# kiranchhatre/amuse

Measured on AMD Instinct MI355X. Metric: SMPL-X frames/sec (10 s clip, 1000-step DDPM), higher is better.
Workload: dtype bf16; 1 GPU; 256 x 10 s clips in total (256 on rank 0), DDPM-1000 sampling loop + VAE decode (300 frames) + 6D->axis-angle; random-init weights of the diff_latent_v2 / prior_emotional_fing architecture; clips_total=256, clips_rank0=256, clips_per_tile=2, sampler=ddpm-1000, mfma_operands=bf16, state_and_accumulate=fp32

## Files before the change

### amuse_amd/csrc/k_vae_fusedx.hip

```cpp
#define AMUSE_OP_F16
#include "amuse_fused.hpp"

namespace amuse {
namespace {

constexpr int kXKvBytes = 4 * kKeyRows * 64;
constexpr int kXOffKv = 0;
constexpr int kXOffW = kXOffKv + kXKvBytes;
constexpr int kXOffPv = kXOffW + kWBufs * kStageBytes;
constexpr int kXOffCa = kXOffPv + 2 * kPvSlot;
constexpr int kXLdsBytes = kXOffCa + kCaBytes;
static_assert(kXLdsBytes <= 160 * 1024, "LDS");
constexpr int kParkTile = 8192;

__device__ __forceinline__ f32x4 mfma3(f16x8 wh, f16x8 wl, const F16Pair& x, f32x4 acc) {
    acc = mfma_f16(wl, x.hi, acc);
    acc = mfma_f16(wh, x.lo, acc);
    return mfma_f16(wh, x.hi, acc);
}
__device__ __forceinline__ f32x4 mfma3t(f16x8 wh, f16x8 wl, const F16Pair& x, f32x4 acc) {
    acc = mfma_f16(x.hi, wl, acc);
    acc = mfma_f16(x.lo, wh, acc);
    return mfma_f16(x.hi, wh, acc);
}
constexpr int kP = 2;
template <int NT>
__device__ __forceinline__ void stage_fetch_x(Stager& s) {
    const unsigned d = __builtin_amdgcn_readfirstlane(s.dst0 + s.widx * kStageBytes);
#pragma unroll
    for (int i = 0; i < kP; ++i) glds16(s.src + i * 64, d + i * 1024);
    s.src += kStage * 64;
    s.widx = s.widx == kWBufs - 1 ? 0 : s.widx + 1;
}
template <int NT>
__device__ __forceinline__ void stage_end_x(Stager& s) {
    asm volatile("s_waitcnt vmcnt(%0) lgkmcnt(0)\n\ts_barrier" ::"n"(kP) : "memory");
    s.ridx = s.ridx == kWBufs - 1 ? 0 : s.ridx + 1;
}
template <int NT, bool FETCH = true, class F>
__device__ __forceinline__ void for_pairs(Stager& s, F&& f) {
    if constexpr (FETCH) stage_fetch_x<NT>(s);
    f16x8 h = wfrag(s, 0), l = wfrag(s, 1);
#pragma unroll
    for (int i = 0; i < 8; ++i) {
        const f16x8 ch = h, cl = l;
        if (i + 1 < 8) { h = wfrag(s, 2 * i + 2); l = wfrag(s, 2 * i + 3); }
        f(i, ch, cl);
    }
}

template <int NT>
struct Images {
    static constexpr int PARK = NT == 3 ? 2 : 0;
    F16Pair reg[NT - PARK][4];
    char* lds;
    __device__ __forceinline__ void build(const f32x4 (&x)[NT][kTiles]) {
#pragma unroll
        for (int j = 0; j < NT; ++j)
#pragma unroll
            for (int c = 0; c < 4; ++c) {
                const F16Pair p = split_f16(x[j][2 * c], x[j][2 * c + 1]);
                if (j < PARK) {
                    *reinterpret_cast<uint4*>(lds + j * kParkTile + (2 * c) * 1024) = __builtin_bit_cast(uint4, p.hi);
                    *reinterpret_cast<uint4*>(lds + j * kParkTile + (2 * c + 1) * 1024) = __builtin_bit_cast(uint4, p.lo);
                } else {
                    reg[j - PARK][c] = p;
                }
            }
    }
    __device__ __forceinline__ F16Pair get(int j, int c) const {
        if (j < PARK) {
            F16Pair p;
            p.hi = __builtin_bit_cast(f16x8, *reinterpret_cast<const uint4*>(lds + j * kParkTile + (2 * c) * 1024));
            p.lo = __builtin_bit_cast(f16x8, *reinterpret_cast<const uint4*>(lds + j * kParkTile + (2 * c + 1) * 1024));
            return p;
        }
        return reg[j - PARK][c];
    }
};

__device__ __forceinline__ void attend_x(const uint4* Kh, const uint4* Kl, const uint4* Vh, const uint4* Vl, const F16Pair& qs, f32x4 (&o)[2], int len, int g, int r) {
    const int fs = frag_slot(g, r);
    o[0] = o[1] = splat4(0.f);
    float m_run = 0.f;
    f32x4 os = splat4(0.f);
    const f16x8 ones = __builtin_bit_cast(f16x8, r == 0 ? uint4{OP_ONE2, OP_ONE2, OP_ONE2, OP_ONE2} : uint4{0u, 0u, 0u, 0u});
    auto pair = [&](int jp, auto first, auto masked) {
        constexpr bool FIRST = decltype(first)::value, MASKED = decltype(masked)::value;
        f16x8 kh[2], kl[2], vh[2], vl[2];
#pragma unroll
        for (int u = 0; u < 2; ++u) {
            kh[u] = __builtin_bit_cast(f16x8, Kh[(2 * jp + u) * 64 + fs]);
            kl[u] = __builtin_bit_cast(f16x8, Kl[(2 * jp + u) * 64 + fs]);
        }
#pragma unroll
        for (int u = 0; u < 2; ++u) {
            vh[u] = __builtin_bit_cast(f16x8, Vh[(2 * jp + u) * 64 + fs]);
            vl[u] = __builtin_bit_cast(f16x8, Vl[(2 * jp + u) * 64 + fs]);
        }
        f32x4 st[2];
        const f32x4 c0 = splat4(-m_run);
#pragma unroll
        for (int u = 0; u < 2; ++u) {
            st[u] = mfma_f16(kl[u], qs.hi, c0);
            st[u] = mfma_f16(kh[u], qs.lo, st[u]);
            st[u] = mfma_f16(kh[u], qs.hi, st[u]);
        }
        if constexpr (MASKED) {
            int lim = len - 32 * jp - 4 * g;
#pragma unroll
            for (int u = 0; u < 2; ++u)
#pragma unroll
                for (int m = 0; m < 4; ++m) st[u][m] = (16 * u + m < lim) ? st[u][m] : -INFINITY;
        }
        float mx = max3(max3(st[0][0], st[0][1], st[0][2]), max3(st[0][3], st[1][0], st[1][1]), fmaxf(st[1][2], st[1][3]));
        if (FIRST || __builtin_amdgcn_ballot_w64(mx > kAttnTau) != 0) {
            mx = allreduce_g_max(mx);
            const float d = FIRST ? mx : fmaxf(mx, 0.f);
            st[0] -= splat4(d);
            st[1] -= splat4(d);
            if constexpr (!FIRST) {
                const float alpha = __builtin_amdgcn_exp2f(-d);
                os *= alpha;
                o[0] *= alpha;
                o[1] *= alpha;
            }
            m_run += d;
        }
        f32x4 p[2];
#pragma unroll
        for (int u = 0; u < 2; ++u)
#pragma unroll
            for (int m = 0; m < 4; ++m) p[u][m] = __builtin_amdgcn_exp2f(st[u][m]);
        const F16Pair pp = split_f16(p[0], p[1]);
#pragma unroll
        for (int td = 0; td < 2; ++td) {
            o[td] = mfma_f16(vl[td], pp.hi, o[td]);
            o[td] = mfma_f16(vh[td], pp.lo, o[td]);
            o[td] = mfma_f16(vh[td], pp.hi, o[td]);
        }
        os = mfma_f16(ones, pp.lo, os);
        os = mfma_f16(ones, pp.hi, os);
    };
    const int full = min(len / 32, kPairs);
    if (full > 0) pair(0, std::true_type{}, std::false_type{});
    else pair(0, std::true_type{}, std::true_type{});
#pragma unroll 1
    for (int jp = 1; jp < full; ++jp) pair(jp, std::false_type{}, std::false_type{});
#pragma unroll 1
    for (int jp = max(full, 1); jp < kPairs; ++jp) pair(jp, std::false_type{}, std::true_type{});
    const float l = allreduce_g_sum(os[0]);
    o[0] = o[0] / l;
    o[1] = o[1] / l;
}

template <class A> struct Geo;
template <> struct Geo<VaeFusedXArgs> {
    static __device__ __forceinline__ int S(const VaeFusedXArgs&) { return kFrames; }
    static __device__ __forceinline__ float* tap(const VaeFusedXArgs& a) { return a.tap_out; }
    static __device__ __forceinline__ const float* c1(const VaeFusedXArgs& a) { return a.c1; }
    static __device__ __forceinline__ float* c1_out(const VaeFusedXArgs& a) { return a.c1_out; }
};
template <> struct Geo<DenFusedXArgs> {
    static __device__ __forceinline__ int S(const DenFusedXArgs& a) { return a.S; }
    static __device__ __forceinline__ float* tap(const DenFusedXArgs&) { return nullptr; }
    static __device__ __forceinline__ const float* c1(const DenFusedXArgs&) { return nullptr; }
    static __device__ __forceinline__ float* c1_out(const DenFusedXArgs&) { return nullptr; }
};

template <int NT, int MODE, class A>
__device__ __forceinline__ void attn_half_x(f32x4 (&x)[NT][kTiles], Stager& sg, const A& a, int b, int blk, int tile0, const float* pv, const float* pv_next_src, unsigned pv_next_dst,
                                            char* smem, int len, int wave, int lane) {
    const int g = lane >> 4, r = lane & 15;
    const int S = Geo<A>::S(a);
    const size_t nrows = (size_t)a.B * S, row0 = (size_t)b * S;
    [[maybe_unused]] const bool prof_on = blockIdx.x == 0 && threadIdx.x == 0 && (blk == 1 || blk == 6);
    FSTAMP(1);
    char* kv = smem + kXOffKv;
    Images<NT> im;
    im.lds = kv + (wave & 3) * (2 * kParkTile) + lane * 16;
    if constexpr (MODE == 2) {
        im.build(x);
        asm volatile("s_waitcnt lgkmcnt(0)" ::: "memory");
        const float* bias = a.pvec + PV_SKIP_B + (blk - 5) * kD;
#pragma unroll
        for (int j = 0; j < NT; ++j)
#pragma unroll
            for (int t = 0; t < kTiles; ++t) x[j][t] = ld4(bias + 16 * t + 4 * g);
#pragma unroll
        for (int c = 0; c < 4; ++c) {
            F16Pair xc[NT];
#pragma unroll
            for (int j = 0; j < NT; ++j) xc[j] = im.get(j, c);
            for_pairs<NT>(sg, [&](int o, f16x8 wh, f16x8 wl) {
#pragma unroll
                for (int j = 0; j < NT; ++j) x[j][o] = mfma3(wh, wl, xc[j], x[j][o]);
            });
            stage_end_x<NT>(sg);
        }
        const float* sk = a.skip + (size_t)(8 - blk) * nrows * kD;
#pragma unroll 1
        for (int c = 0; c < 4; ++c) {
            F16Pair xc[NT];
#pragma unroll
            for (int j = 0; j < NT; ++j) {
                const int frame = 16 * (tile0 + 4 * j) + r;
                const float* src = sk + (row0 + min(frame, S - 1)) * kD + 32 * c + 4 * g;
                const bool ok = frame < S;
                xc[j] = split_f16(ok ? ld4(src) : splat4(0.f), ok ? ld4(src + 16) : splat4(0.f));
            }
            for_pairs<NT>(sg, [&](int o, f16x8 wh, f16x8 wl) {
#pragma unroll
                for (int j = 0; j < NT; ++j) x[j][o] = mfma3(wh, wl, xc[j], x[j][o]);
            });
            stage_end_x<NT>(sg);
        }
    }
    FSTAMP(2);
    {
        uint4* Kh = reinterpret_cast<uint4*>(kv);
        uint4* Kl = Kh + kKeyRows * 4;
        uint4* Vh = Kl + kKeyRows * 4;
        uint4* Vl = Vh + kPairs * 2 * 16 * 4;
        float* obuf = (a.obuf + row0 * kD);
        constexpr float kScaling = 0.17677669529663687f, kLog2e = 1.44269504088896340736f;
#pragma unroll 1
        for (int h = 0; h < kHeads; ++h) {
            {
                f32x4 kk[NT][2], vv[NT][2];
                const f32x4 bk0 = ld4(pv + PV_IN_B + kD + 32 * h + 4 * g), bk1 = ld4(pv + PV_IN_B + kD + 32 * h + 16 + 4 * g);
                const float bv0 = pv[PV_IN_B + 2 * kD + 32 * h + r], bv1 = pv[PV_IN_B + 2 * kD + 32 * h + 16 + r];
#pragma unroll
                for (int j = 0; j < NT; ++j) {
                    kk[j][0] = bk0; kk[j][1] = bk1;
                    vv[j][0] = splat4(bv0); vv[j][1] = splat4(bv1);
                }
#pragma unroll
                for (int s2 = 0; s2 < 2; ++s2) {
                    F16Pair xc[NT];
                    for_pairs<NT>(sg, [&](int i, f16x8 wh, f16x8 wl) {
                        const int c = 2 * s2 + (i >> 2), t = i & 3;
                        if (t == 0) {
#pragma unroll
                            for (int j = 0; j < NT; ++j) xc[j] = split_f16(x[j][2 * c], x[j][2 * c + 1]);
                        }
#pragma unroll
                        for (int j = 0; j < NT; ++j) {
                            if (t < 2) kk[j][t] = mfma3(wh, wl, xc[j], kk[j][t]);
                            else vv[j][t - 2] = mfma3t(wh, wl, xc[j], vv[j][t - 2]);
                        }
                    });
                    if (s2 == 0) stage_end_x<NT>(sg);
                }
                FSTAMP(3);
#pragma unroll
                for (int j = 0; j < NT; ++j) {
                    const int tile = tile0 + 4 * j;
                    const bool ok = 16 * tile + r < S;
                    const F16Pair ks = split_f16(ok ? kk[j][0] : splat4(0.f), ok ? kk[j][1] : splat4(0.f));
                    Kh[tile * 64 + frag_slot(g, r)] = __builtin_bit_cast(uint4, ks.hi);
                    Kl[tile * 64 + frag_slot(g, r)] = __builtin_bit_cast(uint4, ks.lo);
#pragma unroll
                    for (int td = 0; td < 2; ++td) {
                        f32x4 v = vv[j][td];
#pragma unroll
                        for (int m = 0; m < 4; ++m) v[m] = (16 * tile + 4 * g + m < S) ? v[m] : 0.f;
                        const F16Pair vs = split_f16(v, v);
                        const int slot = ((tile >> 1) * 2 + td) * 64 + frag_slot(g, r);
                        const uint4 hi4 = __builtin_bit_cast(uint4, vs.hi), lo4 = __builtin_bit_cast(uint4, vs.lo);
                        *reinterpret_cast<uint2*>(reinterpret_cast<char*>(Vh + slot) + (tile & 1) * 8) = uint2{hi4.x, hi4.y};
                        *reinterpret_cast<uint2*>(reinterpret_cast<char*>(Vl + slot) + (tile & 1) * 8) = uint2{lo4.x, lo4.y};
                    }
                }
                FSTAMP(4);
                stage_end_x<NT>(sg);
                FSTAMP(5);
            }
            if (h == 0 && pv_next_src) {
                const unsigned d = __builtin_amdgcn_readfirstlane(pv_next_dst + wave * 1024);
                glds16(reinterpret_cast<const uint4*>(pv_next_src) + wave * 64 + lane, d);
            }
            F16Pair qs[NT];
            {
                f32x4 q[NT][2];
                const f32x4 bq0 = ld4(pv + PV_IN_B + 32 * h + 4 * g), bq1 = ld4(pv + PV_IN_B + 32 * h + 16 + 4 * g);
#pragma unroll
                for (int j = 0; j < NT; ++j) { q[j][0] = bq0; q[j][1] = bq1; }
                F16Pair xc[NT];
                for_pairs<NT>(sg, [&](int i, f16x8 wh, f16x8 wl) {
                    const int c = i >> 1, o = i & 1;
                    if (o == 0) {
#pragma unroll
                        for (int j = 0; j < NT; ++j) xc[j] = split_f16(x[j][2 * c], x[j][2 * c + 1]);
                    }
#pragma unroll
                    for (int j = 0; j < NT; ++j) q[j][o] = mfma3(wh, wl, xc[j], q[j][o]);
                });
#pragma unroll
                for (int j = 0; j < NT; ++j) qs[j] = split_f16((q[j][0] * kScaling) * kLog2e, (q[j][1] * kScaling) * kLog2e);
            }
            FSTAMP(6);
#pragma unroll 1
            for (int j = 0; j < NT; ++j) {
                f32x4 o[2];
                attend_x(Kh, Kl, Vh, Vl, qs[0], o, len, g, r);
                const int frame = 16 * (tile0 + 4 * j) + r;
                if (frame < S) {
                    float* dst = obuf + (size_t)frame * kD + 32 * h + 4 * g;
                    st4(dst, o[0]);
                    st4(dst + 16, o[1]);
                }
                const F16Pair first = qs[0];
#pragma unroll
                for (int jj = 0; jj + 1 < NT; ++jj) qs[jj] = qs[jj + 1];
                qs[NT - 1] = first;
            }
            FSTAMP(7);
            stage_end_x<NT>(sg);
            FSTAMP(8);
        }
    }
}

template <int NT, int MODE, bool ENCL, class A>
__device__ __forceinline__ void row_half_x(f32x4 (&x)[NT][kTiles], Stager& sg, const A& a, int blk, int tile0, int b, const float* pv, const float* cal, char* smem, int wave,
                                           int lane, const bool hoist = false) {
    const int g = lane >> 4, r = lane & 15;
    const int S = Geo<A>::S(a);
    const size_t nrows = (size_t)a.B * S, row0 = (size_t)b * S;
    [[maybe_unused]] const bool prof_on = blockIdx.x == 0 && threadIdx.x == 0 && (blk == 1 || blk == 6);
    char* kv = smem + kXOffKv;
    Images<NT> im;
    im.lds = kv + (wave & 3) * (2 * kParkTile) + lane * 16;
    if (hoist) {
#pragma unroll
        for (int j = 0; j < NT; ++j) {
            const int frame = 16 * (tile0 + 4 * j) + r;
#pragma unroll
            for (int t = 0; t < kTiles; ++t) x[j][t] = frame < S ? ld4(Geo<A>::c1(a) + (size_t)frame * kD + 16 * t + 4 * g) : splat4(0.f);
        }
    } else {
        float* obuf = (a.obuf + row0 * kD);
#pragma unroll
        for (int j = 0; j < NT; ++j)
#pragma unroll
            for (int t = 0; t < kTiles; ++t) x[j][t] += ld4(pv + PV_OUT_B + 16 * t + 4 * g);
        const unsigned obase = lds_addr(smem) + kXOffKv + (wave < 4 ? wave * 12288 : 49152 + (wave - 4) * 8192);
        const char* obuf_l = smem + kXOffKv + (wave < 4 ? wave * 12288 : 49152 + (wave - 4) * 8192) + lane * 16;
        const float* osrc[NT];
#pragma unroll
        for (int j = 0; j < NT; ++j) osrc[j] = obuf + (size_t)min(16 * (tile0 + 4 * j) + r, S - 1) * kD + 4 * g;
        auto fetch_o = [&](int c) {
            const unsigned d = __builtin_amdgcn_readfirstlane(obase + (c & 1) * (NT * 2048));
#pragma unroll
            for (int j = 0; j < NT; ++j) {
                glds16(reinterpret_cast<const uint4*>(osrc[j] + 32 * c), d + (2 * j) * 1024);
                glds16(reinterpret_cast<const uint4*>(osrc[j] + 32 * c + 16), d + (2 * j + 1) * 1024);
            }
        };
        fetch_o(0);
#pragma unroll 1
        for (int c = 0; c < 4; ++c) {
            stage_fetch_x<NT>(sg);
            if (c + 1 < 4) {
                fetch_o(c + 1);
                asm volatile("s_waitcnt vmcnt(%0)" ::"n"(kP + 2 * NT) : "memory");
            } else {
                asm volatile("s_waitcnt vmcnt(%0)" ::"n"(kP) : "memory");
            }
            F16Pair xc[NT];
#pragma unroll
            for (int j = 0; j < NT; ++j) {
                const char* src = obuf_l + (c & 1) * (NT * 2048) + (2 * j) * 1024;
                xc[j] = split_f16(*reinterpret_cast<const f32x4*>(src), *reinterpret_cast<const f32x4*>(src + 1024));
            }
            for_pairs<NT, false>(sg, [&](int o, f16x8 wh, f16x8 wl) {
#pragma unroll
                for (int j = 0; j < NT; ++j) x[j][o] = mfma3(wh, wl, xc[j], x[j][o]);
            });
            if (c + 1 < 4) {
                asm volatile("s_waitcnt vmcnt(%0) lgkmcnt(0)\n\ts_barrier" ::"n"(kP + 2 * NT) : "memory");
                sg.ridx = sg.ridx == kWBufs - 1 ? 0 : sg.ridx + 1;
            } else {
                stage_end_x<NT>(sg);
            }
            FSTAMP(9);
        }
    }
    {
        const float* ca = cal + blk * kD;
#pragma unroll 1
        for (int j = 0; j < NT; ++j) {
            if (!hoist) layer_norm_rows<false>(x[0], pv + PV_LN1_W, pv + PV_LN1_B, g);
            if (Geo<A>::c1_out(a) && blk == 0 && b == 0) {
                const int frame = 16 * (tile0 + 4 * j) + r;
                if (frame < S) {
#pragma unroll
                    for (int t = 0; t < kTiles; ++t) st4(Geo<A>::c1_out(a) + (size_t)frame * kD + 16 * t + 4 * g, x[0][t]);
                }
            }
            if constexpr (!ENCL) {
#pragma unroll
                for (int t = 0; t < kTiles; ++t) x[0][t] += ld4(ca + 16 * t + 4 * g);
                layer_norm_rows<false>(x[0], pv + PV_LN2_W, pv + PV_LN2_B, g);
            }
            rotate_tiles<NT>(x);
        }
    }
    FSTAMP(10);
    im.build(x);
    asm volatile("s_waitcnt lgkmcnt(0)" ::: "memory");
#pragma unroll
    for (int j = 0; j < NT; ++j)
#pragma unroll
        for (int t = 0; t < kTiles; ++t) x[j][t] += ld4(pv + PV_L2_B + 16 * t + 4 * g);
    f32x4 hid[NT][2];
    auto lin1 = [&](f32x4 (&acc)[NT][2], int ch) {
        const f32x4 b0 = ld4(pv + PV_L1_B + 32 * ch + 4 * g), b1 = ld4(pv + PV_L1_B + 32 * ch + 16 + 4 * g);
#pragma unroll
        for (int j = 0; j < NT; ++j) { acc[j][0] = b0; acc[j][1] = b1; }
        F16Pair xc[NT];
        for_pairs<NT>(sg, [&](int i, f16x8 wh, f16x8 wl) {
            const int c = i >> 1, o = i & 1;
            if (o == 0) {
#pragma unroll
                for (int j = 0; j < NT; ++j) xc[j] = im.get(j, c);
            }
#pragma unroll
            for (int j = 0; j < NT; ++j) {
                acc[j][o] = mfma3(wh, wl, xc[j], acc[j][o]);
            }
        });
    };
    auto gelu_split = [&](F16Pair (&hs)[NT]) {
#pragma unroll
        for (int j = 0; j < NT; ++j) {
#pragma unroll
            for (int i = 0; i < 2; ++i)
#pragma unroll
                for (int m = 0; m < 4; ++m) hid[j][i][m] = gelu_erf_bf(hid[j][i][m]);
            hs[j] = split_f16(hid[j][0], hid[j][1]);
        }
    };
    lin1(hid, 0);
    stage_end_x<NT>(sg);
#pragma unroll 1
    for (int ch = 0; ch < 16; ++ch) {
        F16Pair hs[NT];
        if (ch < 15) {
            f32x4 nxt[NT][2];
            FSTAMP(11);
            if constexpr (NT == 3) {
                lin1(nxt, ch + 1);
                __builtin_amdgcn_sched_barrier(0);
                gelu_split(hs);
            } else {
                gelu_split(hs);
                __builtin_amdgcn_sched_barrier(0);
                lin1(nxt, ch + 1);
            }
            FSTAMP(12);
            stage_end_x<NT>(sg);
            FSTAMP(13);
#pragma unroll
            for (int j = 0; j < NT; ++j) { hid[j][0] = nxt[j][0]; hid[j][1] = nxt[j][1]; }
        } else {
            gelu_split(hs);
        }
        for_pairs<NT>(sg, [&](int o, f16x8 wh, f16x8 wl) {
#pragma unroll
            for (int j = 0; j < NT; ++j) {
                x[j][o] = mfma3(wh, wl, hs[j], x[j][o]);
            }
        });
        FSTAMP(14);
        stage_end_x<NT>(sg);
        FSTAMP(15);
    }
#pragma unroll 1
    for (int j = 0; j < NT; ++j) {
        layer_norm_rows<false>(x[0], pv + (ENCL ? PV_LN2_W : PV_LN3_W), pv + (ENCL ? PV_LN2_B : PV_LN3_B), g);
        rotate_tiles<NT>(x);
    }
    FSTAMP(16);
    if constexpr (MODE == 0) {
        float* sk = a.skip + (size_t)blk * nrows * kD;
#pragma unroll
        for (int j = 0; j < NT; ++j) {
            const int frame = 16 * (tile0 + 4 * j) + r;
            if (frame < S) {
#pragma unroll
                for (int t = 0; t < kTiles; ++t) st4(sk + (row0 + frame) * kD + 16 * t + 4 * g, x[j][t]);
            }
        }
    }
    if (Geo<A>::tap(a) && b == 0) store_tap<NT>(Geo<A>::tap(a), blk, x, tile0, g, r);
}

template <int NT>
__device__ __forceinline__ void decode_tiles_x(const VaeFusedXArgs& a, char* smem, Stager& sg, int tile0, int b, int len, int wave, int lane) {
    const int g = lane >> 4, r = lane & 15;
    const float* pvl = reinterpret_cast<const float*>(smem + kXOffPv);
    const float* cal = reinterpret_cast<const float*>(smem + kXOffCa);
    const unsigned lds0 = lds_addr(smem);
    f32x4 x[NT][kTiles];
#pragma unroll
    for (int j = 0; j < NT; ++j) {
        const int frame = 16 * (tile0 + 4 * j) + r;
#pragma unroll
        for (int t = 0; t < kTiles; ++t) x[j][t] = frame < kFrames ? ld4(a.pe + (size_t)frame * kD + 16 * t + 4 * g) : splat4(0.f);
    }
    asm volatile("s_waitcnt vmcnt(2) lgkmcnt(0)\n\ts_barrier" ::: "memory");
    const bool hoist = a.c1 != nullptr && len == kFrames;
#pragma unroll 1
    for (int blk = 0; blk < 4; ++blk) {
        const float* pv = pvl + (blk & 1) * (kPvSlot / 4);
        const bool h0 = blk == 0 && hoist;
        if (h0) {
            const unsigned d = __builtin_amdgcn_readfirstlane(lds0 + kXOffPv + kPvSlot + wave * 1024);
            glds16(reinterpret_cast<const uint4*>(a.pvec + PV_BLOCK) + wave * 64 + lane, d);
        } else {
            attn_half_x<NT, 0>(x, sg, a, b, blk, tile0, pv, a.pvec + (blk + 1) * PV_BLOCK, lds0 + kXOffPv + ((blk + 1) & 1) * kPvSlot, smem, len, wave, lane);
        }
        row_half_x<NT, 0, false>(x, sg, a, blk, tile0, b, pv, cal, smem, wave, lane, h0);
    }
    attn_half_x<NT, 1>(x, sg, a, b, 4, tile0, pvl, a.pvec + 5 * PV_BLOCK, lds0 + kXOffPv + kPvSlot, smem, len, wave, lane);
    row_half_x<NT, 1, false>(x, sg, a, 4, tile0, b, pvl, cal, smem, wave, lane);
#pragma unroll 1
    for (int blk = 5; blk < kLayers; ++blk) {
        const float* pv = pvl + (blk & 1) * (kPvSlot / 4);
        attn_half_x<NT, 2>(x, sg, a, b, blk, tile0, pv, blk + 1 < kLayers ? a.pvec + (blk + 1) * PV_BLOCK : nullptr, lds0 + kXOffPv + ((blk + 1) & 1) * kPvSlot, smem, len, wave, lane);
        row_half_x<NT, 2, false>(x, sg, a, blk, tile0, b, pv, cal, smem, wave, lane);
    }
#pragma unroll 1
    for (int j = 0; j < NT; ++j) {
        layer_norm_rows<false>(x[0], a.pvec + PV_FINAL_W, a.pvec + PV_FINAL_B, g);
        rotate_tiles<NT>(x);
    }
    if (a.tap_out && b == 0) store_tap<NT>(a.tap_out, 9, x, tile0, g, r);
    F16Pair xs[NT][4];
#pragma unroll
    for (int j = 0; j < NT; ++j)
#pragma unroll
        for (int c = 0; c < 4; ++c) xs[j][c] = split_f16(x[j][2 * c], x[j][2 * c + 1]);
    float* fst = reinterpret_cast<float*>(smem + kXOffKv) + wave * 16 * kQStride;
#pragma unroll 1
    for (int quarter = 0; quarter < 4; ++quarter) {
        f32x4 f[NT][6];
#pragma unroll
        for (int o = 0; o < 6; ++o) {
            const f32x4 bi = ld4(a.final_bias + 16 * (6 * quarter + o) + 4 * g);
#pragma unroll
            for (int j = 0; j < NT; ++j) f[j][o] = bi;
        }
#pragma unroll
        for (int s3 = 0; s3 < 3; ++s3) {
            for_pairs<NT>(sg, [&](int i, f16x8 wh, f16x8 wl) {
                const int lin = 8 * s3 + i, c = lin / 6, o = lin - 6 * c;
#pragma unroll
                for (int j = 0; j < NT; ++j) f[j][o] = mfma3(wh, wl, xs[j][c], f[j][o]);
            });
            stage_end_x<NT>(sg);
        }
        const int f0 = 96 * quarter, nfe = quarter == 3 ? kFeats - 288 : 96, njo = quarter == 3 ? kJoints - 48 : 16;
#pragma unroll 1
        for (int j = 0; j < NT; ++j) {
            const int tile = tile0 + 4 * j;
            const int frame = 16 * tile + r;
            const bool keep = frame < kFrames && frame < len;
            const int rows_here = min(16, kFrames - 16 * tile);
            const size_t row0 = (size_t)b * kFrames + 16 * tile;
#pragma unroll
            for (int o = 0; o < 6; ++o) st4(fst + r * kQStride + 16 * o + 4 * g, keep ? f[0][o] : splat4(0.f));
            asm volatile("s_waitcnt lgkmcnt(0)" ::: "memory");
            if (a.feats_out) {
                for (int i = lane; i < rows_here * nfe; i += 64) {
                    const int rr = i / nfe, c = i - rr * nfe;
                    a.feats_out[(row0 + rr) * kFeats + f0 + c] = fst[rr * kQStride + c];
                }
            }
            if (a.poses_out) {
                for (int i = lane; i < rows_here * njo; i += 64) {
                    const int rr = i / njo, jn = i - rr * njo;
                    float aa[3];
                    rot6d_to_axis_angle(fst + rr * kQStride + 6 * jn, a.quat_mode, aa);
                    float* dst = a.poses_out + ((row0 + rr) * kJoints + 16 * quarter + jn) * 3;
                    dst[0] = aa[0]; dst[1] = aa[1]; dst[2] = aa[2];
                }
            }
            if (a.trans_out && quarter == 3) {
                for (int i = lane; i < rows_here * 3; i += 64) {
                    const int rr = i / 3, c = i - rr * 3;
                    a.trans_out[(row0 + rr) * 3 + c] = fst[rr * kQStride + (330 - 288) + c];
                }
            }
            asm volatile("s_waitcnt lgkmcnt(0)" ::: "memory");
#pragma unroll
            for (int o = 0; o < 6; ++o) {
                const f32x4 first = f[0][o];
#pragma unroll
                for (int jj = 0; jj + 1 < NT; ++jj) f[jj][o] = f[jj + 1][o];
                f[NT - 1][o] = first;
            }
        }
    }
}

__global__ __launch_bounds__(512) __attribute__((amdgpu_waves_per_eu(2, 2))) void k_vae_fusedx(VaeFusedXArgs a) {
    extern __shared__ __attribute__((aligned(16))) char smem[];
    const int lane = threadIdx.x & 63;
    const int wave = __builtin_amdgcn_readfirstlane(threadIdx.x >> 6);
    const int b = blockIdx.x;
    const int len = a.lengths ? a.lengths[b] : kFrames;
    const unsigned lds0 = lds_addr(smem);
    glds16(reinterpret_cast<const uint4*>(a.pvec) + wave * 64 + lane, lds0 + kXOffPv + wave * 1024);
    if (wave < 5) glds16(reinterpret_cast<const uint4*>(a.ca + (size_t)b * kLayers * kD) + wave * 64 + lane, lds0 + kXOffCa + wave * 1024);
    Stager sg;
    const size_t skip_units = (a.c1 && len == kFrames) ? (size_t)16 * kStage : 0;
    const int piece0 = 2 * wave;
    sg.src = a.wstream + (skip_units + (size_t)piece0) * 64 + lane;
    sg.dst0 = lds0 + kXOffW + piece0 * 1024;
    sg.ring = smem + kXOffW + lane * 16;
    sg.widx = 0;
    sg.ridx = 0;
    if (wave < 4) { stage_fetch_x<3>(sg); stage_fetch_x<3>(sg); }
    else { stage_fetch_x<2>(sg); stage_fetch_x<2>(sg); }
    if (wave < 4) decode_tiles_x<3>(a, smem, sg, wave, b, len, wave, lane);
    else decode_tiles_x<2>(a, smem, sg, wave + 8, b, len, wave, lane);
    asm volatile("s_waitcnt vmcnt(0)" ::: "memory");
}

typedef float f32x4u __attribute__((ext_vector_type(4), aligned(4)));
template <int NT>
__device__ __forceinline__ void load_xt_pair(f32x4 (&v)[NT][2], const float* xb, int tile0, int r, int g, int npre, int c) {
#pragma unroll
    for (int j = 0; j < NT; ++j) {
        const int fi = 16 * (tile0 + 4 * j) + r - npre;
        const bool fv = fi >= 0 && fi < kFrames;
        const float* row = xb + (size_t)(fv ? fi : 0) * kFeats + 4 * g;
#pragma unroll
        for (int h = 0; h < 2; ++h) {
            const int f = 32 * c + 16 * h;
            f32x4 t;
            if (f + 15 < kFeats) {
                t = *reinterpret_cast<const f32x4u*>(row + f);
            } else {
#pragma unroll
                for (int m = 0; m < 4; ++m) t[m] = (f + 4 * g + m < kFeats) ? row[f + m] : 0.f;
            }
            v[j][h] = fv ? t : splat4(0.f);
        }
    }
}

template <int NT, bool ENCM>
__device__ __forceinline__ void den_tiles_x(const DenFusedXArgs& a, char* smem, Stager& sg, int tile0, int b, int wave, int lane) {
    const int g = lane >> 4, r = lane & 15;
    const float* pvl = reinterpret_cast<const float*>(smem + kXOffPv);
    const unsigned lds0 = lds_addr(smem);
    const int S = a.S, npre = a.npre;
    const float* xin = a.x_in + (size_t)b * kFrames * kFeats;
    f32x4 x[NT][kTiles];
#pragma unroll
    for (int j = 0; j < NT; ++j)
#pragma unroll
        for (int t = 0; t < kTiles; ++t) x[j][t] = ld4(a.emb_bias + 16 * t + 4 * g);
    f32x4 cur[NT][2];
    load_xt_pair<NT>(cur, xin, tile0, r, g, npre, 0);
    asm volatile("s_waitcnt vmcnt(0) lgkmcnt(0)\n\ts_barrier" ::: "memory");
#pragma unroll 1
    for (int c = 0; c < 11; ++c) {
        F16Pair xc[NT];
#pragma unroll
        for (int j = 0; j < NT; ++j) xc[j] = split_f16(cur[j][0], cur[j][1]);
        if (c + 1 < 11) load_xt_pair<NT>(cur, xin, tile0, r, g, npre, c + 1);
        for_pairs<NT>(sg, [&](int o, f16x8 wh, f16x8 wl) {
#pragma unroll
            for (int j = 0; j < NT; ++j) x[j][o] = mfma3(wh, wl, xc[j], x[j][o]);
        });
        stage_end_x<NT>(sg);
    }
#pragma unroll
    for (int j = 0; j < NT; ++j) {
        const int frame = 16 * (tile0 + 4 * j) + r;
        if constexpr (ENCM) {
#pragma unroll
            for (int t = 0; t < kTiles; ++t) {
                const int c = 16 * t + 4 * g;
                const f32x4 e = frame < npre ? ld4(a.ttok + (frame & 1) * kD + c) : x[j][t];
                x[j][t] = frame < S ? e + ld4(a.pe + (size_t)frame * kD + c) : splat4(0.f);
            }
        } else {
            const float* pt = frame == 0 ? a.ttok + (size_t)b * a.ttok_stride : a.ctok + ((size_t)b * (npre - 1) + (frame < npre ? frame - 1 : 0)) * kD;
#pragma unroll
            for (int t = 0; t < kTiles; ++t) {
                const int c = 16 * t + 4 * g;
                x[j][t] = frame >= S ? splat4(0.f) : (frame < npre ? ld4(pt + c) : x[j][t] + ld4(a.pe + (size_t)frame * kD + c));
            }
        }
    }
    const int klen = ENCM ? (a.lengths ? a.lengths[b] : kFrames) + npre : S;
#pragma unroll 1
    for (int blk = 0; blk < 4; ++blk) {
        const float* pv = pvl + (blk & 1) * (kPvSlot / 4);
        attn_half_x<NT, 0>(x, sg, a, b, blk, tile0, pv, a.pvec + (blk + 1) * PV_BLOCK, lds0 + kXOffPv + ((blk + 1) & 1) * kPvSlot, smem, klen, wave, lane);
        row_half_x<NT, 0, true>(x, sg, a, blk, tile0, b, pv, pvl, smem, wave, lane);
    }
    attn_half_x<NT, 1>(x, sg, a, b, 4, tile0, pvl, a.pvec + 5 * PV_BLOCK, lds0 + kXOffPv + kPvSlot, smem, klen, wave, lane);
    row_half_x<NT, 1, true>(x, sg, a, 4, tile0, b, pvl, pvl, smem, wave, lane);
#pragma unroll 1
    for (int blk = 5; blk < kLayers; ++blk) {
        const float* pv = pvl + (blk & 1) * (kPvSlot / 4);
        attn_half_x<NT, 2>(x, sg, a, b, blk, tile0, pv, blk + 1 < kLayers ? a.pvec + (blk + 1) * PV_BLOCK : nullptr, lds0 + kXOffPv + ((blk + 1) & 1) * kPvSlot, smem, klen, wave, lane);
        row_half_x<NT, 2, true>(x, sg, a, blk, tile0, b, pv, pvl, smem, wave, lane);
    }
    if constexpr (ENCM) {
        if (tile0 == 0) {
            layer_norm_rows<false>(x[0], a.pvec + PV_FINAL_W, a.pvec + PV_FINAL_B, g);
            if (r < 2) {
#pragma unroll
                for (int t = 0; t < kTiles; ++t) st4(a.eps_out + ((size_t)b * 2 + r) * kD + 16 * t + 4 * g, x[0][t]);
            }
        }
        return;
    }
#pragma unroll 1
    for (int j = 0; j < NT; ++j) {
        layer_norm_rows<false>(x[0], a.pvec + PV_FINAL_W, a.pvec + PV_FINAL_B, g);
        rotate_tiles<NT>(x);
    }
    F16Pair xs[NT][4];
#pragma unroll
    for (int j = 0; j < NT; ++j)
#pragma unroll
        for (int c = 0; c < 4; ++c) xs[j][c] = split_f16(x[j][2 * c], x[j][2 * c + 1]);
    float* fst = reinterpret_cast<float*>(smem + kXOffKv) + wave * 16 * kQStride;
    const int len = (a.lengths ? a.lengths[b] : kFrames) + npre;
    const float* cf = a.coef;
    const float sb = cf ? cf[0] : 0.f, sa = cf ? cf[1] : 1.f, c0 = cf ? cf[2] : 0.f, cxx = cf ? cf[3] : 0.f, ce = cf ? cf[4] : 0.f, sgm = cf ? cf[5] : 0.f, clipv = cf ? cf[6] : 0.f;
    const float* nz = a.step_noise ? a.step_noise + (size_t)b * kFrames * kFeats : nullptr;
    float* eo = a.eps_out ? a.eps_out + (size_t)b * kFrames * kFeats : nullptr;
    float* xo = (cf && a.x_out) ? a.x_out + (size_t)b * kFrames * kFeats : nullptr;
#pragma unroll 1
    for (int quarter = 0; quarter < 4; ++quarter) {
        f32x4 f[NT][6];
#pragma unroll
        for (int o = 0; o < 6; ++o) {
            const f32x4 bi = ld4(a.final_bias + 16 * (6 * quarter + o) + 4 * g);
#pragma unroll
            for (int j = 0; j < NT; ++j) f[j][o] = bi;
        }
#pragma unroll
        for (int s3 = 0; s3 < 3; ++s3) {
            for_pairs<NT>(sg, [&](int i, f16x8 wh, f16x8 wl) {
                const int lin = 8 * s3 + i, c = lin / 6, o = lin - 6 * c;
#pragma unroll
                for (int j = 0; j < NT; ++j) f[j][o] = mfma3(wh, wl, xs[j][c], f[j][o]);
            });
            stage_end_x<NT>(sg);
        }
        const int f0 = 96 * quarter, nfe = quarter == 3 ? kFeats - 288 : 96;
#pragma unroll 1
        for (int j = 0; j < NT; ++j) {
            const int tile = tile0 + 4 * j;
            const int frame = 16 * tile + r;
            const bool keep = frame < S && frame < len;
            const int rows_here = min(16, S - 16 * tile);
#pragma unroll
            for (int o = 0; o < 6; ++o) st4(fst + r * kQStride + 16 * o + 4 * g, keep ? f[0][o] : splat4(0.f));
            asm volatile("s_waitcnt lgkmcnt(0)" ::: "memory");
            for (int i = lane; i < rows_here * nfe; i += 64) {
                const int rr = i / nfe, c = i - rr * nfe, fr = 16 * tile + rr - npre;
                if (fr < 0) continue;
                const float e = fst[rr * kQStride + c];
                const size_t el = (size_t)fr * kFeats + f0 + c;
                if (eo) eo[el] = e;
                if (xo) {
#pragma clang fp contract(off)
                    const float xl = xin[el];
                    const float num = __fsub_rn(xl, __fmul_rn(sb, e));
                    float x0 = __fdiv_rn(num, sa);
                    if (clipv > 0.f) x0 = fminf(fmaxf(x0, -clipv), clipv);
                    float nx = __fmul_rn(c0, x0);
                    if (cxx != 0.f) nx = __fadd_rn(nx, __fmul_rn(cxx, xl));
                    if (ce != 0.f) nx = __fadd_rn(nx, __fmul_rn(ce, e));
                    if (sgm != 0.f) {
                        const float z = nz ? nz[el] : counter_normal4(a.seed, a.clip0 + (uint64_t)b, (uint32_t)a.step, (uint32_t)(el >> 2), 1u)[el & 3];
                        nx = __fadd_rn(nx, __fmul_rn(sgm, z));
                    }
                    xo[el] = nx;
                }
            }
            asm volatile("s_waitcnt lgkmcnt(0)" ::: "memory");
#pragma unroll
            for (int o = 0; o < 6; ++o) {
                const f32x4 first = f[0][o];
#pragma unroll
                for (int jj = 0; jj + 1 < NT; ++jj) f[jj][o] = f[jj + 1][o];
                f[NT - 1][o] = first;
            }
        }
    }
}

template <bool ENCM>
__global__ __launch_bounds__(512) __attribute__((amdgpu_waves_per_eu(2, 2))) void k_den_fusedx(DenFusedXArgs a) {
    extern __shared__ __attribute__((aligned(16))) char smem[];
    const int lane = threadIdx.x & 63;
    const int wave = __builtin_amdgcn_readfirstlane(threadIdx.x >> 6);
    const int b = blockIdx.x;
    const unsigned lds0 = lds_addr(smem);
    glds16(reinterpret_cast<const uint4*>(a.pvec) + wave * 64 + lane, lds0 + kXOffPv + wave * 1024);
    Stager sg;
    const int piece0 = 2 * wave;
    sg.src = a.wstream + (size_t)piece0 * 64 + lane;
    sg.dst0 = lds0 + kXOffW + piece0 * 1024;
    sg.ring = smem + kXOffW + lane * 16;
    sg.widx = 0;
    sg.ridx = 0;
    if (wave < 4) { stage_fetch_x<3>(sg); stage_fetch_x<3>(sg); }
    else { stage_fetch_x<2>(sg); stage_fetch_x<2>(sg); }
    if (wave < 4) den_tiles_x<3, ENCM>(a, smem, sg, wave, b, wave, lane);
    else den_tiles_x<2, ENCM>(a, smem, sg, wave + 8, b, wave, lane);
    asm volatile("s_waitcnt vmcnt(0)" ::: "memory");
}

}

hipError_t launch_vae_fusedx(const VaeFusedXArgs& a, hipStream_t stream) {
    static DeviceOnce once;
    int dev_;
    if (!once.done(&dev_)) {
        hipError_t e = hipFuncSetAttribute(reinterpret_cast<const void*>(&k_vae_fusedx), hipFuncAttributeMaxDynamicSharedMemorySize, kXLdsBytes);
        if (e != hipSuccess) return e;
        once.set(dev_);
    }
#if AMUSE_FPROF
    {
        int zero = 0;
        (void)hipMemcpyToSymbol(HIP_SYMBOL(g_fprof_n), &zero, sizeof(int));
    }
#endif
    hipLaunchKernelGGL(k_vae_fusedx, dim3(a.B), dim3(512), kXLdsBytes, stream, a);
#if AMUSE_FPROF
    {
        static int calls = 0;
        (void)hipStreamSynchronize(stream);
        unsigned long long h[512];
        int n = 0;
        (void)hipMemcpyFromSymbol(&n, HIP_SYMBOL(g_fprof_n), sizeof(int));
        (void)hipMemcpyFromSymbol(h, HIP_SYMBOL(g_fprof), sizeof(h));
        if (++calls == 3) {
            for (int i = 1; i < n; ++i) fprintf(stderr, "FPROF %3d tag %2llu  +%llu\n", i, h[2 * i + 1], h[2 * i] - h[2 * i - 2]);
        }
    }
#endif
    return hipGetLastError();
}

hipError_t launch_den_fusedx(const DenFusedXArgs& a, hipStream_t stream) {
    static DeviceOnce once;
    int dev_;
    if (!once.done(&dev_)) {
        for (const void* k : {reinterpret_cast<const void*>(&k_den_fusedx<false>), reinterpret_cast<const void*>(&k_den_fusedx<true>)}) {
            hipError_t e = hipFuncSetAttribute(k, hipFuncAttributeMaxDynamicSharedMemorySize, kXLdsBytes);
            if (e != hipSuccess) return e;
        }
        once.set(dev_);
    }
    if (a.encode) hipLaunchKernelGGL(k_den_fusedx<true>, dim3(a.B), dim3(512), kXLdsBytes, stream, a);
    else hipLaunchKernelGGL(k_den_fusedx<false>, dim3(a.B), dim3(512), kXLdsBytes, stream, a);
    return hipGetLastError();
}

}
```

Measured before the change: 2.231 million frames/s.

## Rematerialize lane index via mbcnt to cut live VGPRs in fused transformer kernels

Stops carrying the lane id and the derived g/r values, plus the per-lane Stager src/ring pointers, through the whole fused denoiser/VAE kernel. Each use site now recomputes the lane with v_mbcnt instructions, which shrinks long-lived VGPR state under the 2-waves-per-EU register budget and should avoid spills. It also moves Images construction into a narrower scope, fully unrolls the skip-add loop, and adds a sched_barrier plus asm register pins around the tile rotation. The cost is a few extra ALU instructions per use, and the added scheduling constraints could hurt instruction interleaving.

```diff
diff --git a/amuse_amd/csrc/k_vae_fusedx.hip b/amuse_amd/csrc/k_vae_fusedx.hip
--- a/amuse_amd/csrc/k_vae_fusedx.hip
+++ b/amuse_amd/csrc/k_vae_fusedx.hip
@@ -13,6 +13,12 @@
 static_assert(kXLdsBytes <= 160 * 1024, "LDS");
 constexpr int kParkTile = 8192;
 
+__device__ __forceinline__ int lane_now() {
+    int l;
+    asm volatile("v_mbcnt_lo_u32_b32 %0, -1, 0\n\tv_mbcnt_hi_u32_b32 %0, -1, %0" : "=v"(l));
+    return l;
+}
+
 __device__ __forceinline__ f32x4 mfma3(f16x8 wh, f16x8 wl, const F16Pair& x, f32x4 acc) {
     acc = mfma_f16(wl, x.hi, acc);
     acc = mfma_f16(wh, x.lo, acc);
@@ -27,8 +33,9 @@
 template <int NT>
 __device__ __forceinline__ void stage_fetch_x(Stager& s) {
     const unsigned d = __builtin_amdgcn_readfirstlane(s.dst0 + s.widx * kStageBytes);
-#pragma unroll
-    for (int i = 0; i < kP; ++i) glds16(s.src + i * 64, d + i * 1024);
+    const uint4* src = s.src + lane_now();
+#pragma unroll
+    for (int i = 0; i < kP; ++i) glds16(src + i * 64, d + i * 1024);
     s.src += kStage * 64;
     s.widx = s.widx == kWBufs - 1 ? 0 : s.widx + 1;
 }
@@ -40,11 +47,13 @@
 template <int NT, bool FETCH = true, class F>
 __device__ __forceinline__ void for_pairs(Stager& s, F&& f) {
     if constexpr (FETCH) stage_fetch_x<NT>(s);
-    f16x8 h = wfrag(s, 0), l = wfrag(s, 1);
+    const char* ring = s.ring + s.ridx * kStageBytes + lane_now() * 16;
+    auto frag = [&](int u) { return __builtin_bit_cast(f16x8, *reinterpret_cast<const uint4*>(ring + u * 1024)); };
+    f16x8 h = frag(0), l = frag(1);
 #pragma unroll
     for (int i = 0; i < 8; ++i) {
         const f16x8 ch = h, cl = l;
-        if (i + 1 < 8) { h = wfrag(s, 2 * i + 2); l = wfrag(s, 2 * i + 3); }
+        if (i + 1 < 8) { h = frag(2 * i + 2); l = frag(2 * i + 3); }
         f(i, ch, cl);
     }
 }
@@ -79,7 +88,8 @@
     }
 };
 
-__device__ __forceinline__ void attend_x(const uint4* Kh, const uint4* Kl, const uint4* Vh, const uint4* Vl, const F16Pair& qs, f32x4 (&o)[2], int len, int g, int r) {
+__device__ __forceinline__ void attend_x(const uint4* Kh, const uint4* Kl, const uint4* Vh, const uint4* Vl, const F16Pair& qs, f32x4 (&o)[2], int len, int lane) {
+    const int g = lane >> 4, r = lane & 15;
     const int fs = frag_slot(g, r);
     o[0] = o[1] = splat4(0.f);
     float m_run = 0.f;
@@ -170,16 +180,16 @@
 
 template <int NT, int MODE, class A>
 __device__ __forceinline__ void attn_half_x(f32x4 (&x)[NT][kTiles], Stager& sg, const A& a, int b, int blk, int tile0, const float* pv, const float* pv_next_src, unsigned pv_next_dst,
-                                            char* smem, int len, int wave, int lane) {
-    const int g = lane >> 4, r = lane & 15;
+                                            char* smem, int len, int wave) {
     const int S = Geo<A>::S(a);
     const size_t nrows = (size_t)a.B * S, row0 = (size_t)b * S;
     [[maybe_unused]] const bool prof_on = blockIdx.x == 0 && threadIdx.x == 0 && (blk == 1 || blk == 6);
     FSTAMP(1);
     char* kv = smem + kXOffKv;
-    Images<NT> im;
-    im.lds = kv + (wave & 3) * (2 * kParkTile) + lane * 16;
     if constexpr (MODE == 2) {
+        const int ls = lane_now(), g = ls >> 4;
+        Images<NT> im;
+        im.lds = kv + (wave & 3) * (2 * kParkTile) + ls * 16;
         im.build(x);
         asm volatile("s_waitcnt lgkmcnt(0)" ::: "memory");
         const float* bias = a.pvec + PV_SKIP_B + (blk - 5) * kD;
@@ -199,8 +209,9 @@
             stage_end_x<NT>(sg);
         }
         const float* sk = a.skip + (size_t)(8 - blk) * nrows * kD;
-#pragma unroll 1
+#pragma unroll
         for (int c = 0; c < 4; ++c) {
+            const int lc = lane_now(), g = lc >> 4, r = lc & 15;
             F16Pair xc[NT];
 #pragma unroll
             for (int j = 0; j < NT; ++j) {
@@ -227,6 +238,7 @@
 #pragma unroll 1
         for (int h = 0; h < kHeads; ++h) {
             {
+                const int lh = lane_now(), g = lh >> 4, r = lh & 15;
                 f32x4 kk[NT][2], vv[NT][2];
                 const f32x4 bk0 = ld4(pv + PV_IN_B + kD + 32 * h + 4 * g), bk1 = ld4(pv + PV_IN_B + kD + 32 * h + 16 + 4 * g);
                 const float bv0 = pv[PV_IN_B + 2 * kD + 32 * h + r], bv1 = pv[PV_IN_B + 2 * kD + 32 * h + 16 + r];
@@ -278,10 +290,11 @@
             }
             if (h == 0 && pv_next_src) {
                 const unsigned d = __builtin_amdgcn_readfirstlane(pv_next_dst + wave * 1024);
-                glds16(reinterpret_cast<const uint4*>(pv_next_src) + wave * 64 + lane, d);
+                glds16(reinterpret_cast<const uint4*>(pv_next_src) + wave * 64 + lane_now(), d);
             }
             F16Pair qs[NT];
             {
+                const int g = lane_now() >> 4;
                 f32x4 q[NT][2];
                 const f32x4 bq0 = ld4(pv + PV_IN_B + 32 * h + 4 * g), bq1 = ld4(pv + PV_IN_B + 32 * h + 16 + 4 * g);
 #pragma unroll
@@ -303,7 +316,8 @@
 #pragma unroll 1
             for (int j = 0; j < NT; ++j) {
                 f32x4 o[2];
-                attend_x(Kh, Kl, Vh, Vl, qs[0], o, len, g, r);
+                const int lt = lane_now(), g = lt >> 4, r = lt & 15;
+                attend_x(Kh, Kl, Vh, Vl, qs[0], o, len, lt);
                 const int frame = 16 * (tile0 + 4 * j) + r;
                 if (frame < S) {
                     float* dst = obuf + (size_t)frame * kD + 32 * h + 4 * g;
@@ -324,15 +338,13 @@
 
 template <int NT, int MODE, bool ENCL, class A>
 __device__ __forceinline__ void row_half_x(f32x4 (&x)[NT][kTiles], Stager& sg, const A& a, int blk, int tile0, int b, const float* pv, const float* cal, char* smem, int wave,
-                                           int lane, const bool hoist = false) {
-    const int g = lane >> 4, r = lane & 15;
+                                           const bool hoist = false) {
     const int S = Geo<A>::S(a);
     const size_t nrows = (size_t)a.B * S, row0 = (size_t)b * S;
     [[maybe_unused]] const bool prof_on = blockIdx.x == 0 && threadIdx.x == 0 && (blk == 1 || blk == 6);
     char* kv = smem + kXOffKv;
-    Images<NT> im;
-    im.lds = kv + (wave & 3) * (2 * kParkTile) + lane * 16;
     if (hoist) {
+        const int lh = lane_now(), g = lh >> 4, r = lh & 15;
 #pragma unroll
         for (int j = 0; j < NT; ++j) {
             const int frame = 16 * (tile0 + 4 * j) + r;
@@ -340,13 +352,14 @@
             for (int t = 0; t < kTiles; ++t) x[j][t] = frame < S ? ld4(Geo<A>::c1(a) + (size_t)frame * kD + 16 * t + 4 * g) : splat4(0.f);
         }
     } else {
+        const int lo = lane_now(), g = lo >> 4, r = lo & 15;
         float* obuf = (a.obuf + row0 * kD);
 #pragma unroll
         for (int j = 0; j < NT; ++j)
 #pragma unroll
             for (int t = 0; t < kTiles; ++t) x[j][t] += ld4(pv + PV_OUT_B + 16 * t + 4 * g);
         const unsigned obase = lds_addr(smem) + kXOffKv + (wave < 4 ? wave * 12288 : 49152 + (wave - 4) * 8192);
-        const char* obuf_l = smem + kXOffKv + (wave < 4 ? wave * 12288 : 49152 + (wave - 4) * 8192) + lane * 16;
+        const char* obuf_l = smem + kXOffKv + (wave < 4 ? wave * 12288 : 49152 + (wave - 4) * 8192) + lo * 16;
         const float* osrc[NT];
 #pragma unroll
         for (int j = 0; j < NT; ++j) osrc[j] = obuf + (size_t)min(16 * (tile0 + 4 * j) + r, S - 1) * kD + 4 * g;
@@ -391,6 +404,8 @@
         const float* ca = cal + blk * kD;
 #pragma unroll 1
         for (int j = 0; j < NT; ++j) {
+            const int ln = lane_now(), g = ln >> 4;
+            [[maybe_unused]] const int r = ln & 15;
             if (!hoist) layer_norm_rows<false>(x[0], pv + PV_LN1_W, pv + PV_LN1_B, g);
             if (Geo<A>::c1_out(a) && blk == 0 && b == 0) {
                 const int frame = 16 * (tile0 + 4 * j) + r;
@@ -404,18 +419,29 @@
                 for (int t = 0; t < kTiles; ++t) x[0][t] += ld4(ca + 16 * t + 4 * g);
                 layer_norm_rows<false>(x[0], pv + PV_LN2_W, pv + PV_LN2_B, g);
             }
+            __builtin_amdgcn_sched_barrier(0);
             rotate_tiles<NT>(x);
+#pragma unroll
+            for (int jj = 0; jj < NT; ++jj)
+#pragma unroll
+                for (int t = 0; t < kTiles; ++t) asm volatile("" : "+v"(x[jj][t]));
         }
     }
     FSTAMP(10);
-    im.build(x);
-    asm volatile("s_waitcnt lgkmcnt(0)" ::: "memory");
-#pragma unroll
-    for (int j = 0; j < NT; ++j)
-#pragma unroll
-        for (int t = 0; t < kTiles; ++t) x[j][t] += ld4(pv + PV_L2_B + 16 * t + 4 * g);
+    Images<NT> im;
+    {
+        const int lf = lane_now(), g = lf >> 4;
+        im.lds = kv + (wave & 3) * (2 * kParkTile) + lf * 16;
+        im.build(x);
+        asm volatile("s_waitcnt lgkmcnt(0)" ::: "memory");
+#pragma unroll
+        for (int j = 0; j < NT; ++j)
+#pragma unroll
+            for (int t = 0; t < kTiles; ++t) x[j][t] += ld4(pv + PV_L2_B + 16 * t + 4 * g);
+    }
     f32x4 hid[NT][2];
     auto lin1 = [&](f32x4 (&acc)[NT][2], int ch) {
+        const int g = lane_now() >> 4;
         const f32x4 b0 = ld4(pv + PV_L1_B + 32 * ch + 4 * g), b1 = ld4(pv + PV_L1_B + 32 * ch + 16 + 4 * g);
 #pragma unroll
         for (int j = 0; j < NT; ++j) { acc[j][0] = b0; acc[j][1] = b1; }
@@ -479,10 +505,12 @@
     }
 #pragma unroll 1
     for (int j = 0; j < NT; ++j) {
+        const int g = lane_now() >> 4;
         layer_norm_rows<false>(x[0], pv + (ENCL ? PV_LN2_W : PV_LN3_W), pv + (ENCL ? PV_LN2_B : PV_LN3_B), g);
         rotate_tiles<NT>(x);
     }
     FSTAMP(16);
+    const int le = lane_now(), g = le >> 4, r = le & 15;
     if constexpr (MODE == 0) {
         float* sk = a.skip + (size_t)blk * nrows * kD;
 #pragma unroll
@@ -498,14 +526,14 @@
 }
 
 template <int NT>
-__device__ __forceinline__ void decode_tiles_x(const VaeFusedXArgs& a, char* smem, Stager& sg, int tile0, int b, int len, int wave, int lane) {
-    const int g = lane >> 4, r = lane & 15;
+__device__ __forceinline__ void decode_tiles_x(const VaeFusedXArgs& a, char* smem, Stager& sg, int tile0, int b, int len, int wave) {
     const float* pvl = reinterpret_cast<const float*>(smem + kXOffPv);
     const float* cal = reinterpret_cast<const float*>(smem + kXOffCa);
     const unsigned lds0 = lds_addr(smem);
     f32x4 x[NT][kTiles];
 #pragma unroll
     for (int j = 0; j < NT; ++j) {
+        const int l0 = lane_now(), g = l0 >> 4, r = l0 & 15;
         const int frame = 16 * (tile0 + 4 * j) + r;
 #pragma unroll
         for (int t = 0; t < kTiles; ++t) x[j][t] = frame < kFrames ? ld4(a.pe + (size_t)frame * kD + 16 * t + 4 * g) : splat4(0.f);
@@ -518,26 +546,26 @@
         const bool h0 = blk == 0 && hoist;
         if (h0) {
             const unsigned d = __builtin_amdgcn_readfirstlane(lds0 + kXOffPv + kPvSlot + wave * 1024);
-            glds16(reinterpret_cast<const uint4*>(a.pvec + PV_BLOCK) + wave * 64 + lane, d);
+            glds16(reinterpret_cast<const uint4*>(a.pvec + PV_BLOCK) + wave * 64 + lane_now(), d);
         } else {
-            attn_half_x<NT, 0>(x, sg, a, b, blk, tile0, pv, a.pvec + (blk + 1) * PV_BLOCK, lds0 + kXOffPv + ((blk + 1) & 1) * kPvSlot, smem, len, wave, lane);
-        }
-        row_half_x<NT, 0, false>(x, sg, a, blk, tile0, b, pv, cal, smem, wave, lane, h0);
-    }
-    attn_half_x<NT, 1>(x, sg, a, b, 4, tile0, pvl, a.pvec + 5 * PV_BLOCK, lds0 + kXOffPv + kPvSlot, smem, len, wave, lane);
-    row_half_x<NT, 1, false>(x, sg, a, 4, tile0, b, pvl, cal, smem, wave, lane);
+            attn_half_x<NT, 0>(x, sg, a, b, blk, tile0, pv, a.pvec + (blk + 1) * PV_BLOCK, lds0 + kXOffPv + ((blk + 1) & 1) * kPvSlot, smem, len, wave);
+        }
+        row_half_x<NT, 0, false>(x, sg, a, blk, tile0, b, pv, cal, smem, wave, h0);
+    }
+    attn_half_x<NT, 1>(x, sg, a, b, 4, tile0, pvl, a.pvec + 5 * PV_BLOCK, lds0 + kXOffPv + kPvSlot, smem, len, wave);
+    row_half_x<NT, 1, false>(x, sg, a, 4, tile0, b, pvl, cal, smem, wave);
 #pragma unroll 1
     for (int blk = 5; blk < kLayers; ++blk) {
         const float* pv = pvl + (blk & 1) * (kPvSlot / 4);
-        attn_half_x<NT, 2>(x, sg, a, b, blk, tile0, pv, blk + 1 < kLayers ? a.pvec + (blk + 1) * PV_BLOCK : nullptr, lds0 + kXOffPv + ((blk + 1) & 1) * kPvSlot, smem, len, wave, lane);
-        row_half_x<NT, 2, false>(x, sg, a, blk, tile0, b, pv, cal, smem, wave, lane);
+        attn_half_x<NT, 2>(x, sg, a, b, blk, tile0, pv, blk + 1 < kLayers ? a.pvec + (blk + 1) * PV_BLOCK : nullptr, lds0 + kXOffPv + ((blk + 1) & 1) * kPvSlot, smem, len, wave);
+        row_half_x<NT, 2, false>(x, sg, a, blk, tile0, b, pv, cal, smem, wave);
     }
 #pragma unroll 1
     for (int j = 0; j < NT; ++j) {
-        layer_norm_rows<false>(x[0], a.pvec + PV_FINAL_W, a.pvec + PV_FINAL_B, g);
+        layer_norm_rows<false>(x[0], a.pvec + PV_FINAL_W, a.pvec + PV_FINAL_B, lane_now() >> 4);
         rotate_tiles<NT>(x);
     }
-    if (a.tap_out && b == 0) store_tap<NT>(a.tap_out, 9, x, tile0, g, r);
+    if (a.tap_out && b == 0) store_tap<NT>(a.tap_out, 9, x, tile0, lane_now() >> 4, lane_now() & 15);
     F16Pair xs[NT][4];
 #pragma unroll
     for (int j = 0; j < NT; ++j)
@@ -547,6 +575,7 @@
 #pragma unroll 1
     for (int quarter = 0; quarter < 4; ++quarter) {
         f32x4 f[NT][6];
+        const int g = lane_now() >> 4;
 #pragma unroll
         for (int o = 0; o < 6; ++o) {
             const f32x4 bi = ld4(a.final_bias + 16 * (6 * quarter + o) + 4 * g);
@@ -565,6 +594,7 @@
         const int f0 = 96 * quarter, nfe = quarter == 3 ? kFeats - 288 : 96, njo = quarter == 3 ? kJoints - 48 : 16;
 #pragma unroll 1
         for (int j = 0; j < NT; ++j) {
+            const int lt = lane_now(), g = lt >> 4, r = lt & 15;
             const int tile = tile0 + 4 * j;
             const int frame = 16 * tile + r;
             const bool keep = frame < kFrames && frame < len;
@@ -574,13 +604,13 @@
             for (int o = 0; o < 6; ++o) st4(fst + r * kQStride + 16 * o + 4 * g, keep ? f[0][o] : splat4(0.f));
             asm volatile("s_waitcnt lgkmcnt(0)" ::: "memory");
             if (a.feats_out) {
-                for (int i = lane; i < rows_here * nfe; i += 64) {
+                for (int i = lt; i < rows_here * nfe; i += 64) {
                     const int rr = i / nfe, c = i - rr * nfe;
                     a.feats_out[(row0 + rr) * kFeats + f0 + c] = fst[rr * kQStride + c];
                 }
             }
             if (a.poses_out) {
-                for (int i = lane; i < rows_here * njo; i += 64) {
+                for (int i = lt; i < rows_here * njo; i += 64) {
                     const int rr = i / njo, jn = i - rr * njo;
                     float aa[3];
                     rot6d_to_axis_angle(fst + rr * kQStride + 6 * jn, a.quat_mode, aa);
@@ -589,7 +619,7 @@
                 }
             }
             if (a.trans_out && quarter == 3) {
-                for (int i = lane; i < rows_here * 3; i += 64) {
+                for (int i = lt; i < rows_here * 3; i += 64) {
                     const int rr = i / 3, c = i - rr * 3;
                     a.trans_out[(row0 + rr) * 3 + c] = fst[rr * kQStride + (330 - 288) + c];
                 }
@@ -618,15 +648,15 @@
     Stager sg;
     const size_t skip_units = (a.c1 && len == kFrames) ? (size_t)16 * kStage : 0;
     const int piece0 = 2 * wave;
-    sg.src = a.wstream + (skip_units + (size_t)piece0) * 64 + lane;
+    sg.src = a.wstream + (skip_units + (size_t)piece0) * 64;
     sg.dst0 = lds0 + kXOffW + piece0 * 1024;
-    sg.ring = smem + kXOffW + lane * 16;
+    sg.ring = smem + kXOffW;
     sg.widx = 0;
     sg.ridx = 0;
     if (wave < 4) { stage_fetch_x<3>(sg); stage_fetch_x<3>(sg); }
     else { stage_fetch_x<2>(sg); stage_fetch_x<2>(sg); }
-    if (wave < 4) decode_tiles_x<3>(a, smem, sg, wave, b, len, wave, lane);
-    else decode_tiles_x<2>(a, smem, sg, wave + 8, b, len, wave, lane);
+    if (wave < 4) decode_tiles_x<3>(a, smem, sg, wave, b, len, wave);
+    else decode_tiles_x<2>(a, smem, sg, wave + 8, b, len, wave);
     asm volatile("s_waitcnt vmcnt(0)" ::: "memory");
 }
 
@@ -654,8 +684,8 @@
 }
 
 template <int NT, bool ENCM>
-__device__ __forceinline__ void den_tiles_x(const DenFusedXArgs& a, char* smem, Stager& sg, int tile0, int b, int wave, int lane) {
-    const int g = lane >> 4, r = lane & 15;
+__device__ __forceinline__ void den_tiles_x(const DenFusedXArgs& a, char* smem, Stager& sg, int tile0, int b, int wave) {
+    const int l0 = lane_now(), g = l0 >> 4, r = l0 & 15;
     const float* pvl = reinterpret_cast<const float*>(smem + kXOffPv);
     const unsigned lds0 = lds_addr(smem);
     const int S = a.S, npre = a.npre;
@@ -670,6 +700,7 @@
     asm volatile("s_waitcnt vmcnt(0) lgkmcnt(0)\n\ts_barrier" ::: "memory");
 #pragma unroll 1
     for (int c = 0; c < 11; ++c) {
+        const int lc = lane_now(), g = lc >> 4, r = lc & 15;
         F16Pair xc[NT];
 #pragma unroll
         for (int j = 0; j < NT; ++j) xc[j] = split_f16(cur[j][0], cur[j][1]);
@@ -682,6 +713,7 @@
     }
 #pragma unroll
     for (int j = 0; j < NT; ++j) {
+        const int lj = lane_now(), g = lj >> 4, r = lj & 15;
         const int frame = 16 * (tile0 + 4 * j) + r;
         if constexpr (ENCM) {
 #pragma unroll
@@ -703,19 +735,20 @@
 #pragma unroll 1
     for (int blk = 0; blk < 4; ++blk) {
         const float* pv = pvl + (blk & 1) * (kPvSlot / 4);
-        attn_half_x<NT, 0>(x, sg, a, b, blk, tile0, pv, a.pvec + (blk + 1) * PV_BLOCK, lds0 + kXOffPv + ((blk + 1) & 1) * kPvSlot, smem, klen, wave, lane);
-        row_half_x<NT, 0, true>(x, sg, a, blk, tile0, b, pv, pvl, smem, wave, lane);
-    }
-    attn_half_x<NT, 1>(x, sg, a, b, 4, tile0, pvl, a.pvec + 5 * PV_BLOCK, lds0 + kXOffPv + kPvSlot, smem, klen, wave, lane);
-    row_half_x<NT, 1, true>(x, sg, a, 4, tile0, b, pvl, pvl, smem, wave, lane);
+        attn_half_x<NT, 0>(x, sg, a, b, blk, tile0, pv, a.pvec + (blk + 1) * PV_BLOCK, lds0 + kXOffPv + ((blk + 1) & 1) * kPvSlot, smem, klen, wave);
+        row_half_x<NT, 0, true>(x, sg, a, blk, tile0, b, pv, pvl, smem, wave);
+    }
+    attn_half_x<NT, 1>(x, sg, a, b, 4, tile0, pvl, a.pvec + 5 * PV_BLOCK, lds0 + kXOffPv + kPvSlot, smem, klen, wave);
+    row_half_x<NT, 1, true>(x, sg, a, 4, tile0, b, pvl, pvl, smem, wave);
 #pragma unroll 1
     for (int blk = 5; blk < kLayers; ++blk) {
         const float* pv = pvl + (blk & 1) * (kPvSlot / 4);
-        attn_half_x<NT, 2>(x, sg, a, b, blk, tile0, pv, blk + 1 < kLayers ? a.pvec + (blk + 1) * PV_BLOCK : nullptr, lds0 + kXOffPv + ((blk + 1) & 1) * kPvSlot, smem, klen, wave, lane);
-        row_half_x<NT, 2, true>(x, sg, a, blk, tile0, b, pv, pvl, smem, wave, lane);
+        attn_half_x<NT, 2>(x, sg, a, b, blk, tile0, pv, blk + 1 < kLayers ? a.pvec + (blk + 1) * PV_BLOCK : nullptr, lds0 + kXOffPv + ((blk + 1) & 1) * kPvSlot, smem, klen, wave);
+        row_half_x<NT, 2, true>(x, sg, a, blk, tile0, b, pv, pvl, smem, wave);
     }
     if constexpr (ENCM) {
         if (tile0 == 0) {
+            const int lz = lane_now(), g = lz >> 4, r = lz & 15;
             layer_norm_rows<false>(x[0], a.pvec + PV_FINAL_W, a.pvec + PV_FINAL_B, g);
             if (r < 2) {
 #pragma unroll
@@ -726,7 +759,7 @@
     }
 #pragma unroll 1
     for (int j = 0; j < NT; ++j) {
-        layer_norm_rows<false>(x[0], a.pvec + PV_FINAL_W, a.pvec + PV_FINAL_B, g);
+        layer_norm_rows<false>(x[0], a.pvec + PV_FINAL_W, a.pvec + PV_FINAL_B, lane_now() >> 4);
         rotate_tiles<NT>(x);
     }
     F16Pair xs[NT][4];
@@ -744,6 +777,7 @@
 #pragma unroll 1
     for (int quarter = 0; quarter < 4; ++quarter) {
         f32x4 f[NT][6];
+        const int g = lane_now() >> 4;
 #pragma unroll
         for (int o = 0; o < 6; ++o) {
             const f32x4 bi = ld4(a.final_bias + 16 * (6 * quarter + o) + 4 * g);
@@ -762,6 +796,7 @@
         const int f0 = 96 * quarter, nfe = quarter == 3 ? kFeats - 288 : 96;
 #pragma unroll 1
         for (int j = 0; j < NT; ++j) {
+            const int lt = lane_now(), g = lt >> 4, r = lt & 15;
             const int tile = tile0 + 4 * j;
             const int frame = 16 * tile + r;
             const bool keep = frame < S && frame < len;
@@ -769,7 +804,7 @@
 #pragma unroll
             for (int o = 0; o < 6; ++o) st4(fst + r * kQStride + 16 * o + 4 * g, keep ? f[0][o] : splat4(0.f));
             asm volatile("s_waitcnt lgkmcnt(0)" ::: "memory");
-            for (int i = lane; i < rows_here * nfe; i += 64) {
+            for (int i = lt; i < rows_here * nfe; i += 64) {
                 const int rr = i / nfe, c = i - rr * nfe, fr = 16 * tile + rr - npre;
                 if (fr < 0) continue;
                 const float e = fst[rr * kQStride + c];
@@ -813,15 +848,15 @@
     glds16(reinterpret_cast<const uint4*>(a.pvec) + wave * 64 + lane, lds0 + kXOffPv + wave * 1024);
     Stager sg;
     const int piece0 = 2 * wave;
-    sg.src = a.wstream + (size_t)piece0 * 64 + lane;
+    sg.src = a.wstream + (size_t)piece0 * 64;
     sg.dst0 = lds0 + kXOffW + piece0 * 1024;
-    sg.ring = smem + kXOffW + lane * 16;
+    sg.ring = smem + kXOffW;
     sg.widx = 0;
     sg.ridx = 0;
     if (wave < 4) { stage_fetch_x<3>(sg); stage_fetch_x<3>(sg); }
     else { stage_fetch_x<2>(sg); stage_fetch_x<2>(sg); }
-    if (wave < 4) den_tiles_x<3, ENCM>(a, smem, sg, wave, b, wave, lane);
-    else den_tiles_x<2, ENCM>(a, smem, sg, wave + 8, b, wave, lane);
+    if (wave < 4) den_tiles_x<3, ENCM>(a, smem, sg, wave, b, wave);
+    else den_tiles_x<2, ENCM>(a, smem, sg, wave + 8, b, wave);
     asm volatile("s_waitcnt vmcnt(0)" ::: "memory");
 }
 
```

Result: no change. 2.229 million frames/s (median of 2 runs) (-0.1%).
